# alexv879/ClusterMachineLearningForHospitalNetworks-Apache-Spark

Measured on AMD Instinct MI355X. Metric: KMeans fit samples/sec (whole node), 100M×256 k=256 at 1/2/4/8 MI355X, higher is better.
Workload: dtype bf16; 1 GPU; model=KMeans k=256, 100000000x256, global_batch=100000000, parallelism=dp1, k=256, rows=100000000, dim=256

## Files before the change

clustermachinelearningforhospitalnetworks_apache_spark_amd/_native/csrc/kmeans.hip:

```cpp
#include <algorithm>

#include "common.h"

namespace {

constexpr int kAccumThreads = 1024;
constexpr int kSegThreads = 256;

template <int DP>
struct AssignShape {
  static constexpr int NCH = DP / 8;
  static constexpr int KS = DP >= 32 ? DP / 32 : 1;
};
constexpr int kAssignThreads = 512;

template <bool HI>
__device__ __forceinline__ unsigned f8x2_to_bf16x2(unsigned w) {
  typedef float f2 __attribute__((ext_vector_type(2)));
  const f2 v = __builtin_amdgcn_cvt_pk_f32_fp8((int)w, HI);
  return (__float_as_uint(v.x) >> 16) | (__float_as_uint(v.y) & 0xffff0000u);
}

template <int DP, bool F8>
__device__ __forceinline__ void load_x16(const void* __restrict__ Xv, long long n, long long ldx, long long row0,
// ... 457 lines not shown
    msg[kd + c] = (double)tot[c];
    carry = base;
    if (c == k - 1) {
      seg[k] = (int)(base + tot[c]);
      double cs = 0.0;
      for (int i = 0; i < ncost; ++i) cs += cost_part[i];
      msg[kd + k] = cs;
    }
  }
  __syncthreads();
  for (int b0 = 0; b0 < nblk; b0 += blockDim.x) {
    const int b = b0 + tid;
    const long long v = b < nblk ? hist[(long long)b * kp + c] : 0;
    long long incl = v;
#pragma unroll
    for (int o = 1; o < 64; o <<= 1) {
      const long long y = __shfl_up(incl, o, 64);
      if (lane >= o) incl += y;
    }
    __syncthreads();
    if (lane == 63) ws[wave] = incl;
    __syncthreads();
    long long pre = carry;
    for (int w = 0; w < wave; ++w) pre += ws[w];
    if (b < nblk) off[(long long)c * nblk + b] = (int)(pre + incl - v);
    __syncthreads();
    if (tid == blockDim.x - 1) carry = pre + incl;
    __syncthreads();
  }
}

constexpr int kScatterThreads = 512;
constexpr int kScatterU = 4;
__global__ __launch_bounds__(kScatterThreads) void kmeans_scatter(const int* __restrict__ labels,
                                                                  const int* __restrict__ rank, long long n, int nblk,
                                                                  int nwaves, int tile_rows, int k,
                                                                  const int* __restrict__ off, int* __restrict__ perm,
                                                                  const int* __restrict__ gate, int want) {
  extern __shared__ int soff[];
  if (gate != nullptr && gate[0] != want) return;
  const int b = blockIdx.x;
  for (int c = threadIdx.x; c < k; c += blockDim.x) soff[c] = off[(long long)c * nblk + b];
  __syncthreads();
  const long long grp = (long long)nwaves * tile_rows;
  const long long stride = grp * nblk;
  const int per = (long long)blockDim.x >= grp ? (int)(blockDim.x / grp) : 1;
  const int ro = per > 1 ? (int)(threadIdx.x / grp) : 0;
  if (ro >= per) return;
  const long long o0 = per > 1 ? (long long)threadIdx.x - ro * grp : (long long)threadIdx.x;
  const long long ostep = per > 1 ? grp : (long long)blockDim.x;
  for (long long q0 = ro; (long long)b * grp + q0 * stride < n; q0 += (long long)per * kScatterU) {
    for (long long o = o0; o < grp; o += ostep) {
      int lab[kScatterU], rk[kScatterU];
      long long rows[kScatterU];
#pragma unroll
      for (int u = 0; u < kScatterU; ++u) {
        rows[u] = (long long)b * grp + (q0 + (long long)u * per) * stride + o;
        lab[u] = rows[u] < n ? labels[rows[u]] : -1;
        rk[u] = rows[u] < n ? rank[rows[u]] : 0;
      }
#pragma unroll
      for (int u = 0; u < kScatterU; ++u)
        if (lab[u] >= 0) {
          const long long pos = (long long)soff[lab[u]] + rk[u];
          if (pos < n) perm[pos] = (int)rows[u];
        }
    }
  }
}

template <int CPL> struct RawCols;
template <> struct RawCols<2> { using T = unsigned; };
template <> struct RawCols<4> { using T = uint2; };
template <> struct RawCols<8> { using T = uint4; };

template <int CPL>
__device__ __forceinline__ void add_raw(double (&acc)[CPL], const typename RawCols<CPL>::T& w) {
  const unsigned* ws = reinterpret_cast<const unsigned*>(&w);
#pragma unroll
  for (int q = 0; q < CPL / 2; ++q) {
    acc[2 * q] += (double)bf16_to_f32((u16)(ws[q] & 0xffffu));
    acc[2 * q + 1] += (double)bf16_to_f32((u16)(ws[q] >> 16));
  }
}

template <int CPL>
__device__ __forceinline__ void add_raw_q(double (&acc)[CPL], const typename RawCols<CPL>::T& w, double qs,
                                          float qsf) {
  const unsigned* ws = reinterpret_cast<const unsigned*>(&w);
  if (qsf != 0.f) {
#pragma unroll
    for (int q = 0; q < CPL / 2; ++q) {
      acc[2 * q] += (double)rintf(bf16_to_f32((u16)(ws[q] & 0xffffu)) * qsf);
      acc[2 * q + 1] += (double)rintf(bf16_to_f32((u16)(ws[q] >> 16)) * qsf);
    }
  } else {
#pragma unroll
    for (int q = 0; q < CPL / 2; ++q) {
      acc[2 * q] += rint((double)bf16_to_f32((u16)(ws[q] & 0xffffu)) * qs);
// ... 68 lines not shown
      s = fmaf(e0, e0, s);
      s = fmaf(e1, e1, s);
    }
  }
  return s;
}

__device__ __forceinline__ float wave_total_dpp(float v) {
  v += __int_as_float(__builtin_amdgcn_update_dpp(0, __float_as_int(v), 0xB1, 0xf, 0xf, false));
  v += __int_as_float(__builtin_amdgcn_update_dpp(0, __float_as_int(v), 0x4E, 0xf, 0xf, false));
  v += __int_as_float(__builtin_amdgcn_update_dpp(0, __float_as_int(v), 0x141, 0xf, 0xf, false));
  v += __int_as_float(__builtin_amdgcn_update_dpp(0, __float_as_int(v), 0x140, 0xf, 0xf, false));
  v += __int_as_float(__builtin_amdgcn_update_dpp(0, __float_as_int(v), 0x142, 0xa, 0xf, false));
  v += __int_as_float(__builtin_amdgcn_update_dpp(0, __float_as_int(v), 0x143, 0xc, 0xf, false));
  return __int_as_float(__builtin_amdgcn_readlane(__float_as_int(v), 63));
}

__device__ __forceinline__ float batch16_totals(const float (&s)[16]) {
  const int lane = threadIdx.x & 63;
  const bool h5 = lane & 32, h4 = lane & 16, h3 = lane & 8, h2 = lane & 4;
  float a[8], b[4], c[2];
#pragma unroll
  for (int i = 0; i < 8; ++i) a[i] = (h5 ? s[8 + i] : s[i]) + __shfl_xor(h5 ? s[i] : s[8 + i], 32, 64);
#pragma unroll
  for (int i = 0; i < 4; ++i) b[i] = (h4 ? a[4 + i] : a[i]) + __shfl_xor(h4 ? a[i] : a[4 + i], 16, 64);
#pragma unroll
  for (int i = 0; i < 2; ++i) c[i] = (h3 ? b[2 + i] : b[i]) + __shfl_xor(h3 ? b[i] : b[2 + i], 8, 64);
  float v = (h2 ? c[1] : c[0]) + __shfl_xor(h2 ? c[0] : c[1], 4, 64);
  v += __int_as_float(__builtin_amdgcn_update_dpp(0, __float_as_int(v), 0xB1, 0xf, 0xf, false));
  v += __int_as_float(__builtin_amdgcn_update_dpp(0, __float_as_int(v), 0x4E, 0xf, 0xf, false));
  return __shfl(v, 4 * (lane & 15), 64);
}

struct SegUB {
  const u16* cb;
  long long ldc;
  float* ub;
  double qs;
  const float* cu = nullptr;
};

__device__ __forceinline__ long long seg_chunk(long long filled, long long waves) {
  const long long c = (filled + waves - 1) / waves;
  return c > 128 ? c : 128;
}

template <int CPL, bool F8, bool UB = false, bool Q = false>
__global__ __launch_bounds__(kSegThreads, (CPL <= 4 ? 4 : 1)) void kmeans_segacc(const void* __restrict__ X, long long n, long long ldx,
                                                             int Dp, int D, const int* __restrict__ perm,
                                                             const int* __restrict__ seg, int k,
                                                             double* __restrict__ msg, double* __restrict__ slots,
                                                             int* __restrict__ slot_c, const int* __restrict__ gate,
                                                             int want, SegUB sub) {
  using raw_t = typename SegRaw<CPL, F8>::T;
  constexpr int U = 16;
  if (gate != nullptr && gate[0] != want) return;
  const unsigned char* xb = reinterpret_cast<const unsigned char*>(X);
  constexpr int ESZ = F8 ? 1 : 2;
  const int lane = threadIdx.x & 63;
  const long long wave = (long long)blockIdx.x * (kSegThreads / 64) + (threadIdx.x >> 6);
  n = n < (long long)seg[k] ? n : (long long)seg[k];
  const long long chunk = seg_chunk(n, (long long)gridDim.x * (kSegThreads / 64));
  const long long p0 = wave * chunk;
  if (p0 >= n) {
    if (lane == 0) {
      slot_c[2 * wave] = -1;
      slot_c[2 * wave + 1] = -1;
    }
    return;
  }
  double* slotA = slots + (2 * wave) * (long long)D;
  double* slotB = slotA + D;
  int nflush = 0;
  const long long p1 = p0 + chunk < n ? p0 + chunk : n;
  int lo = 0, hi = k;
  while (hi - lo > 1) {
    const int mid = (lo + hi) >> 1;
    if (seg[mid] <= p0) lo = mid; else hi = mid;
  }
  int c = lo;
  long long next = seg[c + 1];
  while (next <= p0) { ++c; next = seg[c + 1]; }
  const int col = CPL * lane;
  const bool active = col < Dp;
  double acc[CPL];
#pragma unroll
  for (int j = 0; j < CPL; ++j) acc[j] = 0.0;
  float cv[CPL];
  auto load_cv = [&](int cc) {
#pragma unroll
    for (int j = 0; j < CPL; ++j) cv[j] = active ? bf16_to_f32(sub.cb[(long long)cc * sub.ldc + col + j]) : 0.f;
  };
  if constexpr (UB) load_cv(c);
  const float qsf = grid_scale_f32(sub.qs);
  auto ub_of = [](float s) { return sqrtf(s * (1.0f + 1.0f / 8192.0f)) * (1.0f + 1e-6f); };
  auto ub_store = [&](float u, int cc) {
    if (sub.cu == nullptr) return u;
    const float cu = sub.cu[cc];
    return (u - cu) + 1e-6f * (u + cu);
  };
  int pr_next = (lane < U && p0 + lane < p1) ? perm[p0 + lane] : 0;
  for (long long p = p0; p < p1; p += U) {
    const int cnt = (int)(p1 - p < U ? p1 - p : U);
    const int pr = pr_next;
    pr_next = (lane < U && p + U + lane < p1) ? perm[p + U + lane] : 0;
    float mine = 0.f;
    raw_t w[U];
#pragma unroll
    for (int u = 0; u < U; ++u) {
      const long long row = __builtin_amdgcn_readlane(pr, u);
      if (u < cnt && active) {
        w[u] = *reinterpret_cast<const raw_t*>(xb + (row * ldx + col) * ESZ);
      } else {
        w[u] = raw_t{};
      }
    }
    const long long pe = p + cnt;
    if (next >= pe) {
      if constexpr (UB) {
        static_assert(U == 16, "batch16_totals");
        if constexpr (CPL <= 8) {
          float sq[U];
#pragma unroll
          for (int u = 0; u < U; ++u) sq[u] = sqdist_raw<CPL, F8>(w[u], cv);
          mine = batch16_totals(sq);
        } else {
#pragma unroll
          for (int u = 0; u < U; ++u) {
            const float t = wave_total_dpp(sqdist_raw<CPL, F8>(w[u], cv));
            mine = lane == u ? t : mine;
          }
        }
        if (lane < cnt) sub.ub[pr] = ub_store(ub_of(mine), c);
      }
      if constexpr (F8) {
        float part[CPL];
#pragma unroll
        for (int j = 0; j < CPL; ++j) part[j] = 0.f;
#pragma unroll
        for (int u = 0; u < U; ++u) add_raw8_f32<CPL>(part, w[u]);
#pragma unroll
        for (int j = 0; j < CPL; ++j) acc[j] += (double)part[j];
      } else {
#pragma unroll
        for (int u = 0; u < U; ++u) {
          if constexpr (Q) add_raw_q<CPL>(acc, w[u], sub.qs, qsf);
          else add_raw<CPL>(acc, w[u]);
        }
      }
    } else {
      int rc = c;
#pragma unroll 1
      for (int u = 0; u < cnt; ++u) {
        const long long pos = p + u;
        while (pos >= next) {
          double* dst = nflush == 0 ? slotA : msg + (long long)c * D;
          if (active) {
#pragma unroll
            for (int j = 0; j < CPL; ++j)
              if (col + j < D) dst[col + j] = acc[j];
          }
          if (nflush == 0 && lane == 0) slot_c[2 * wave] = c;
          ++nflush;
#pragma unroll
          for (int j = 0; j < CPL; ++j) acc[j] = 0.0;
          ++c;
          next = seg[c + 1];
          while (next <= pos && c < k - 1) { ++c; next = seg[c + 1]; }
          if constexpr (UB) load_cv(c);
        }
        const long long row = __builtin_amdgcn_readlane(pr, u);
        raw_t v = raw_t{};
        if (active) v = *reinterpret_cast<const raw_t*>(xb + (row * ldx + col) * ESZ);
        if constexpr (UB) {
          const float t = wave_total_dpp(sqdist_raw<CPL, F8>(v, cv));
          mine = lane == u ? t : mine;
          rc = lane == u ? c : rc;
        }
        if constexpr (F8) add_raw8<CPL>(acc, v);
        else if constexpr (Q) add_raw_q<CPL>(acc, v, sub.qs, qsf);
        else add_raw<CPL>(acc, v);
      }
      if constexpr (UB) {
        if (lane < cnt) sub.ub[pr] = ub_store(ub_of(mine), rc);
      }
    }
  }
  if (active) {
#pragma unroll
    for (int j = 0; j < CPL; ++j)
      if (col + j < D) slotB[col + j] = acc[j];
  }
  if (lane == 0) {
    if (nflush == 0) slot_c[2 * wave] = -1;
    slot_c[2 * wave + 1] = c;
  }
}

__device__ __forceinline__ float init_reach(float cost, float xn, float pn, float tau) {
  return 2.0f * sqrtf(fmaxf(cost, 0.f) + tau * (xn + pn)) * (1.0f + 2e-6f);
}

constexpr int kClsPer = 16;
constexpr int kClsRows = 256 * kClsPer;

__global__ __launch_bounds__(256) void init_classify_kernel(const float* __restrict__ cost,
                                                            const int* __restrict__ near, const float* __restrict__ xn,
                                                            const float* __restrict__ pn,
                                                            const float* __restrict__ tab_v, int m, float tau,
                                                            long long n, int lmax, int* __restrict__ list_a,
                                                            int* __restrict__ cnt_a, int* __restrict__ list_b,
                                                            int* __restrict__ cnt_b) {
  __shared__ int wa[4], wb[4], base[2];
  const int lane = threadIdx.x & 63, wv = threadIdx.x >> 6;
  for (long long c0 = (long long)blockIdx.x * kClsRows; c0 < n; c0 += (long long)gridDim.x * kClsRows) {
    unsigned cls = 0;
#pragma unroll
// ... 446 lines not shown
int launch_assign(const void* X, long long n, long long ldx, const u16* C, long long ldc, int kc, int kp,
                  int c_base, const float* cnorm, const float* xnorm, int* labels, float* best, int first, int last,
                  double* cost_part, int* hist, int* rank, DeltaOut dout, int grid, hipStream_t st) {
  const size_t lds = (size_t)assign_lds_bytes(kc, kp, DP);
  const void* fn = assign_kernel_ptr<DP, F8>();
  hipFuncSetAttribute(fn, hipFuncAttributeMaxDynamicSharedMemorySize, (int)lds);
  void* args[] = {(void*)&X, (void*)&n, (void*)&ldx, (void*)&C, (void*)&ldc, (void*)&kc, (void*)&kp,
                  (void*)&c_base, (void*)&cnorm, (void*)&xnorm, (void*)&labels, (void*)&best, (void*)&first,
                  (void*)&last, (void*)&cost_part, (void*)&hist, (void*)&rank, (void*)&dout};
  const hipError_t e = hipLaunchKernel(fn, dim3(grid), dim3(kAssignThreads), args, lds, st);
  if (e != hipSuccess) return (int)e;
  return cml_status();
}

long long priv_lds_bytes(int k, int dw, int rpw) {
  const long long NW = kAccumThreads / 64;
  return NW * rpw * k * dw * 4 + NW * rpw * k * 4;
}

template <int CPL, int RPW>
int launch_priv(const u16* X, long long n, long long ldx, const int* labels, int k, int dw, float* slab, int* cslab,
                int gx, int nsl, hipStream_t st) {
  const size_t lds = (size_t)priv_lds_bytes(k, dw, RPW);
  hipFuncSetAttribute((const void*)kmeans_accum_priv<CPL, RPW>, hipFuncAttributeMaxDynamicSharedMemorySize, (int)lds);
  hipLaunchKernelGGL((kmeans_accum_priv<CPL, RPW>), dim3(gx, nsl), dim3(kAccumThreads), lds, st, X, n, ldx, labels, k,
                     dw, slab, cslab);
  return cml_status();
}

int launch_segsum(const void* X, long long n, long long ldx, int Dp, int D, const int* perm, const int* seg, int k,
                  int cpl, int seg_grid, double* msg, double* slots, int* slot_c, int xfp8, const int* gate, int want,
                  hipStream_t st, SegUB sub = SegUB{nullptr, 0, nullptr, 0.0}, bool fixup = true) {
  const long long waves = (long long)seg_grid * (kSegThreads / 64);
#define CML_SEG_L(C, F, U, Q)                                                                                       \
  hipLaunchKernelGGL((kmeans_segacc<C, F, U, Q>), dim3(seg_grid), dim3(kSegThreads), 0, st, X, n, ldx, Dp, D, perm, \
                     seg, k, msg, slots, slot_c, gate, want, sub)
#define CML_SEG(C, F)                                                  \
  if (sub.ub != nullptr) {                                             \
    if (!F && sub.qs != 0.0) CML_SEG_L(C, F, true, !F);               \
    else CML_SEG_L(C, F, true, false);                                 \
  } else {                                                             \
    if (!F && sub.qs != 0.0) CML_SEG_L(C, F, false, !F);              \
    else CML_SEG_L(C, F, false, false);                                \
  }
  if (xfp8) {
    if (cpl == 4) CML_SEG(4, true)
    else if (cpl == 8) CML_SEG(8, true)
    else if (cpl == 16) CML_SEG(16, true)
    else return (int)hipErrorInvalidValue;
  } else if (cpl == 2) CML_SEG(2, false)
  else if (cpl == 4) CML_SEG(4, false)
  else if (cpl == 8) CML_SEG(8, false)
  else return (int)hipErrorInvalidValue;
#undef CML_SEG
#undef CML_SEG_L
  const int e = cml_status();
  if (e || !fixup) return e;
  hipLaunchKernelGGL(kmeans_seg_fixup, dim3(k), dim3(256), 0, st, seg, k, D, n, waves, slots, slot_c, msg, gate,
                     want);
  return cml_status();
}

}

CML_API long long cml_kmeans_assign_lds_bytes(int kc, int kp, int Dp) { return assign_lds_bytes(kc, kp, Dp); }
CML_API int cml_kmeans_assign_threads(int ) { return kAssignThreads; }
CML_API int cml_kmeans_assign_occupancy(int Dp, int kc, int kp, int xfp8) {
  if (xfp8) {
    switch (Dp) {
      case 64: return assign_occupancy<64, true>(kc, kp);
      case 128: return assign_occupancy<128, true>(kc, kp);
      case 256: return assign_occupancy<256, true>(kc, kp);
      case 512: return assign_occupancy<512, true>(kc, kp);
      default: return 0;
    }
  }
// ... 143 lines not shown
  CML_PRIV(2, 1); CML_PRIV(2, 2); CML_PRIV(2, 4); CML_PRIV(2, 8); CML_PRIV(2, 16);
  CML_PRIV(4, 1); CML_PRIV(4, 2); CML_PRIV(4, 4); CML_PRIV(4, 8); CML_PRIV(4, 16);
#undef CML_PRIV
  return (int)hipErrorInvalidValue;
}

CML_API int cml_kmeans_reduce(const float* slab, const int* cslab, const double* cost_part, int gx, int ncost, int k,
                              int D, int dsl, double* out, void* stream) {
  const long long total = (long long)k * D + k + 1;
  const int threads = 256;
  const long long blocks = (total + threads - 1) / threads;
  hipLaunchKernelGGL(kmeans_reduce_kernel, dim3((unsigned)blocks), dim3(threads), 0, (hipStream_t)stream, slab, cslab,
                     cost_part, gx, ncost, k, D, dsl, out);
  return cml_status();
}

static int sort_accum(const void* X, long long n, long long ldx, int Dp, int D, const int* labels, const int* rank,
                      const int* hist, int nblk, int round_rows, int k, int kp, const double* cost_part, int ncost,
                      int* off, int* seg, int* perm, int cpl, int seg_grid, double* msg, double* slots, int* slot_c,
                      int xfp8, const int* gate, void* stream, SegUB sub);
CML_API int cml_kmeans_sort_accum(const void* X, long long n, long long ldx, int Dp, int D, const int* labels,
                                  const int* rank, const int* hist, int nblk, int round_rows, int k, int kp,
                                  const double* cost_part, int ncost, int* off, int* seg, int* perm, int cpl,
                                  int seg_grid, double* msg, double* slots, int* slot_c, int xfp8, const int* gate,
                                  double qscale, void* stream) {
  return sort_accum(X, n, ldx, Dp, D, labels, rank, hist, nblk, round_rows, k, kp, cost_part, ncost, off, seg, perm,
                    cpl, seg_grid, msg, slots, slot_c, xfp8, gate, stream, SegUB{nullptr, 0, nullptr, qscale});
}
CML_API int cml_kmeans_sort_accum_ub(const void* X, long long n, long long ldx, int Dp, int D, const int* labels,
                                     const int* rank, const int* hist, int nblk, int round_rows, int k, int kp,
                                     const double* cost_part, int ncost, int* off, int* seg, int* perm, int cpl,
                                     int seg_grid, double* msg, double* slots, int* slot_c, int xfp8, const int* gate,
                                     const void* cb, long long ldc, float* ub, double qscale, const float* cu,
                                     void* stream) {
  if (cb == nullptr || ub == nullptr || ldc < Dp) return (int)hipErrorInvalidValue;
  return sort_accum(X, n, ldx, Dp, D, labels, rank, hist, nblk, round_rows, k, kp, cost_part, ncost, off, seg, perm,
                    cpl, seg_grid, msg, slots, slot_c, xfp8, gate, stream, SegUB{(const u16*)cb, ldc, ub, qscale, cu});
}
static int sort_accum(const void* X, long long n, long long ldx, int Dp, int D, const int* labels, const int* rank,
                      const int* hist, int nblk, int round_rows, int k, int kp, const double* cost_part, int ncost,
                      int* off, int* seg, int* perm, int cpl, int seg_grid, double* msg, double* slots, int* slot_c,
                      int xfp8, const int* gate, void* stream, SegUB sub) {
  hipStream_t st = (hipStream_t)stream;
  long long* tot = reinterpret_cast<long long*>(seg + k + 1 + ((k + 1) & 1));
  const int want = 1;
  if (gate == nullptr) {
    hipMemsetAsync(msg, 0, sizeof(double) * (size_t)k * D, st);
  } else {
    hipLaunchKernelGGL(zero_f64_gated, dim3(256), dim3(256), 0, st, msg, (long long)k * D, gate, want);
  }
  hipLaunchKernelGGL(kmeans_seg_totals, dim3(k), dim3(256), 0, st, hist, nblk, kp, tot, gate, want);
  hipLaunchKernelGGL(kmeans_seg_offsets, dim3(k), dim3(256), 0, st, hist, nblk, k, kp, tot, cost_part, ncost, D, off,
                     seg, msg, gate, want);
  int e = cml_status();
  if (e) return e;
  if (n == 0) return 0;
  hipLaunchKernelGGL(kmeans_scatter, dim3(nblk), dim3(kScatterThreads), sizeof(int) * (size_t)k, st,
                     labels, rank, n,
                     nblk, 1, round_rows, k, off, perm, gate, want);
  e = cml_status();
  if (e) return e;
  return launch_segsum(X, n, ldx, Dp, D, perm, seg, k, cpl, seg_grid, msg, slots, slot_c, xfp8, gate, want, st, sub);
}

CML_API int cml_kmeans_sort_perm(long long n, const int* labels, const int* rank, const int* hist, int nblk,
                                 int round_rows, int k, int kp, const double* cost_part, int ncost, int* off, int* seg,
                                 int* perm, double* tail, void* stream) {
  if (k <= 0 || nblk <= 0 || n < 0 || tail == nullptr) return (int)hipErrorInvalidValue;
  hipStream_t st = (hipStream_t)stream;
  long long* tot = reinterpret_cast<long long*>(seg + k + 1 + ((k + 1) & 1));
  hipLaunchKernelGGL(kmeans_seg_totals, dim3(k), dim3(256), 0, st, hist, nblk, kp, tot, (const int*)nullptr, 1);
  hipLaunchKernelGGL(kmeans_seg_offsets, dim3(k), dim3(256), 0, st, hist, nblk, k, kp, tot, cost_part,
                     cost_part != nullptr ? ncost : 0, 0, off, seg, tail, (const int*)nullptr, 1);
  int e = cml_status();
  if (e || n == 0) return e;
  hipLaunchKernelGGL(kmeans_scatter, dim3(nblk), dim3(kScatterThreads), sizeof(int) * (size_t)k, st, labels, rank, n,
                     nblk, 1, round_rows, k, off, perm, (const int*)nullptr, 1);
  return cml_status();
}

CML_API int cml_kmeans_delta_gate(const int* chg_wg_count, int nblk, int cap, int* chg_overflow, int* force, int* mode,
                                  int k, int* dh, void* stream) {
  hipLaunchKernelGGL(kmeans_delta_gate, dim3(1), dim3(256), 0, (hipStream_t)stream, chg_wg_count, nblk, cap,
                     chg_overflow, force, mode, k, dh);
  return cml_status();
}

CML_API int cml_kmeans_delta_accum(const void* X, long long ldx, int Dp, int D, const int* labels, const int* chg_rows,
                                   const int* chg_old, const int* chg_wg_count, int nblk, int pcap, int cap,
                                   const int* mode, int k, int* dh, int* dseg,
                                   int* cursor, int* dperm, int cpl, int seg_grid, double* dsum, double* slots,
                                   int* slot_c, double* acc, const double* cost_part, int ncost, double* msg, int xfp8,
                                   double qscale, void* stream) {
  hipStream_t st = (hipStream_t)stream;
  const size_t lh = sizeof(int) * 2 * (size_t)k;
  hipLaunchKernelGGL(kmeans_delta_hist, dim3(nblk), dim3(kDeltaThreads), lh, st, chg_rows, chg_old, labels,
                     chg_wg_count, pcap, mode, k, dh, dsum, 2LL * k * D, cursor);
  hipLaunchKernelGGL(kmeans_delta_scatter, dim3(nblk), dim3(kDeltaThreads), lh + sizeof(int) * (2 * (size_t)k + 1), st,
                     chg_rows, chg_old, labels, chg_wg_count, pcap, mode, k, cursor, dperm, dh, dseg);
  int e = cml_status();
  if (e) return e;
  if (cap > 0) {
    e = launch_segsum(X, 2LL * cap, ldx, Dp, D, dperm, dseg, 2 * k, cpl, seg_grid, dsum, slots, slot_c, xfp8, mode, 0,
                      st, SegUB{nullptr, 0, nullptr, qscale}, false);
    if (e) return e;
  }
  const long long total = (long long)k * D + k + 1;
  const long long waves = (long long)seg_grid * (kSegThreads / 64);
  hipLaunchKernelGGL(kmeans_delta_apply, dim3((unsigned)((total + 255) / 256)), dim3(256), 0, st, acc, dsum, dseg,
                     mode, k, D, cost_part, ncost, msg, cap > 0 ? slots : nullptr, slot_c, 2LL * cap, waves);
// ... 61 lines not shown
```

clustermachinelearningforhospitalnetworks_apache_spark_amd/models/kmeans.py:

```python
from __future__ import annotations

import math
import os
import types
from typing import List, Optional

import numpy as np
import torch

from .. import _native
from ..ops import kmeans_ops as K
from ..ops.group_ops import group_reduce
from ..parallel.comm import Communicator, local_comm
from ..utils import rng
from ..utils.device import padded_dim, round_up
from ..utils.fault import maybe_fail
from ..utils.trace import trace


def padded_dim_fp8(d: int) -> int:
    return max(256, 1 << max(0, (d - 1).bit_length()))


def to_device_matrix(x: torch.Tensor, d: Optional[int] = None) -> torch.Tensor:
# ... 1006 lines not shown
        if self._conv_lim is not None:
            K.converge_latch(self.shift2, k, self._conv_lim, st.flags)

    def _seed_from_init(self, sd) -> None:
        st, n, k, d = self._pst, self.n, self.k, self.d
        if n == 0:
            return
        U = sd.uniq.to(device=self.device, dtype=torch.float64)
        a, d1, d2, pn32 = K.seed_table(U, self.cb, k)
        qmap = sd.inverse.reshape(-1).to(torch.int32).contiguous()
        if st.cum is not None:
            st.cum.zero_()
        K.seed_bounds(sd.nearest[:n], sd.costs[:n], self.xnorm[:n], qmap, a, d1, d2, pn32, 2.0 * self._tau, n,
                      self.labels[:n], st.ub[:n], st.lb[:n])

    def _step_seeded(self) -> None:
        st, dl = self._pst, self.delta
        n, k, d, ap = self.n, self.k, self.d, self.aplan
        x, lab, msg = self.x, self.labels, self.msgs[0]
        if n:
            K.prune_bounds(lab, st.ub, st.lb, st.drift, st.dmax, st.thr, st.c2, k, st.cand, st.count,
                           xn=self.xnorm, cand_lab=st.cand_lab, cand_xn=st.cand_xn, zero_count=True, cum=st.cum)
            K.prune_gate(st.count, st.cap_m, st.flags, st.pmode)
            K.assign_rr_ext(1, x, n, self.dp, self.cb, self.cnorm, ap, self.xnorm, lab, self.cost_part, st.ub, st.lb,
                            st.mc, st.tau, hist=self.hist, rank=self.rank, delta=dl, gate=st.pmode, want=1,
                            cum=st.cum)
            K.assign_rr_ext(2, x, st.cap_m, self.dp, self.cb, self.cnorm, ap, st.cand_xn, lab, None, st.ub, st.lb,
                            st.mc, st.tau, delta=dl, idx=st.cand, n_dev=st.count, lab_in=st.cand_lab, gate=st.pmode,
                            want=0, cum=st.cum)
            K.label_hist(lab, n, ap, self.hist, self.rank, gate=st.pmode, want=0)
        self.cost_part.zero_()
        dl.invalidate()
        dl.gate(0)
        K.accumulate_sort(x, n, self.dp, d, lab, self.rank, self.hist, ap, k, self.cost_part, self.off, self.seg,
                          self.perm, self.cplan, dl.acc[0], self.slots, gate=dl.mode[0],
                          ub_centres=self.cb, ub=st.ub, qscale=self._qscale, cum=st.cum)
        dl.accumulate(x, self.dp, lab, 0, self.cost_part, ap.grid, msg, qscale=self._qscale)
        self.comm.allreduce_async(msg).wait()
        self._pdev_post()

    def _norms64(self) -> torch.Tensor:
        self._ensure_norms()
        if self._xnorm64 is None:
            self._xnorm64 = torch.empty(max(self.n, 1), dtype=torch.float64, device=self.device)
            if self.n:
                tmp = torch.empty(self.n, dtype=torch.float32, device=self.device)
                for _, r0, r1, xc in self._x_chunks(whole=True):
                    K.row_pass(xc, r1 - r0, self.dp, tmp[r0:r1], xn64=self._xnorm64[r0:r1])
        return self._xnorm64

    def _device_cost(self) -> torch.Tensor:
        k, d, n = self.k, self.d, self.n
        cb = self._pst.cb_cost if self._pdev else self._cb_cost
        if k <= 4096:
            bound = self._xmax_dev()
            limbs = torch.zeros(2 * k, dtype=torch.int64, device=self.device)
            if n:
                lab = self.labels[:n]
                lab = lab if lab.dtype == torch.int32 and lab.is_contiguous() else lab.to(torch.int32).contiguous()
                K.fixsum(self._norms64()[:n], n, bound, 1.0, lab=lab, k=k, limbs=limbs)
            self.comm.allreduce_(limbs)
            q = K.fixsum_finalize(limbs, k, bound, 1.0)
        else:
            if n:
                q = group_reduce(self.labels[:n], self._norms64()[:n], k, "sum",
                                 ids_in_range=True).to(torch.float64).contiguous()
            else:
                q = torch.zeros(k, dtype=torch.float64, device=self.device)
            self.comm.allreduce_(q)
# ... 829 lines not shown
```

clustermachinelearningforhospitalnetworks_apache_spark_amd/ops/kmeans_ops.py:

```python
from __future__ import annotations

import ctypes
import os
import threading

from dataclasses import dataclass

import torch

from .. import _native
from .._native import c_dbl, c_int, c_ll, c_vp
from ..utils.device import LDS_BUDGET, num_cus, round_up

_native.register_kernel_sigs({
    "cml_kmeans_assign_lds_bytes": (c_ll, [c_int, c_int, c_int]),
    "cml_kmeans_assign_threads": (c_int, [c_int]),
    "cml_kmeans_set_assign_variant": (c_int, [c_int]),
    "cml_kmeans_assign_occupancy": (c_int, [c_int, c_int, c_int, c_int]),
    "cml_kmeans_seg_threads": (c_int, []),
    "cml_kmeans_seg_ints": (c_ll, [c_int]),
    "cml_kmeans_assign_bf16": (c_int, [c_vp, c_ll, c_ll, c_int, c_vp, c_ll, c_int, c_int, c_int, c_vp, c_vp, c_vp,
                                       c_vp, c_int, c_int, c_vp, c_vp, c_vp, c_int, c_int, c_vp, c_vp, c_vp, c_vp,
                                       c_int, c_int, c_vp]),
    "cml_kmeans_assign_rr_plan": (c_int, [c_int, c_int, c_int, c_int, c_vp]),
    "cml_kmeans_set_rr_default": (c_int, [c_int]),
    "cml_kmeans_set_rr_debug": (c_int, [c_int]),
    "cml_kmeans_set_rr_m32": (c_int, [c_int]),
    "cml_kmeans_set_fp8_mx": (c_int, [c_int]),
    "cml_kmeans_assign_tile_rows": (c_int, [c_int]),
    "cml_row_sqnorm_bf16": (c_int, [c_vp, c_ll, c_ll, c_int, c_vp, c_vp]),
    "cml_row_sqnorm_fp8": (c_int, [c_vp, c_ll, c_ll, c_int, c_vp, c_vp]),
    "cml_kmeans_priv_lds_bytes": (c_ll, [c_int, c_int, c_int]),
    "cml_kmeans_accum_priv": (c_int, [c_vp, c_ll, c_ll, c_vp, c_int, c_int, c_int, c_int, c_vp, c_vp, c_int, c_int,
                                      c_vp]),
    "cml_kmeans_reduce": (c_int, [c_vp, c_vp, c_vp, c_int, c_int, c_int, c_int, c_int, c_vp, c_vp]),
    "cml_kmeans_sort_accum": (c_int, [c_vp, c_ll, c_ll, c_int, c_int, c_vp, c_vp, c_vp, c_int, c_int, c_int, c_int,
                                      c_vp, c_int, c_vp, c_vp, c_vp, c_int, c_int, c_vp, c_vp, c_vp, c_int, c_vp,
                                      ctypes.c_double, c_vp]),
    "cml_kmeans_sort_accum_ub": (c_int, [c_vp, c_ll, c_ll, c_int, c_int, c_vp, c_vp, c_vp, c_int, c_int, c_int,
                                         c_int, c_vp, c_int, c_vp, c_vp, c_vp, c_int, c_int, c_vp, c_vp, c_vp, c_int,
                                         c_vp, c_vp, c_ll, c_vp, ctypes.c_double, c_vp, c_vp]),
    "cml_kmeans_delta_gate": (c_int, [c_vp, c_int, c_int, c_vp, c_vp, c_vp, c_int, c_vp, c_vp]),
    "cml_kmeans_delta_accum": (c_int, [c_vp, c_ll, c_int, c_int, c_vp, c_vp, c_vp, c_vp, c_int, c_int, c_int, c_vp,
                                       c_int, c_vp, c_vp, c_vp, c_vp, c_int, c_int, c_vp, c_vp, c_vp, c_vp, c_vp,
                                       c_int, c_vp, c_int, ctypes.c_double, c_vp]),
    "cml_kmeans_seg_slot_doubles": (c_ll, [c_int, c_int]),
    "cml_kmeans_seg_slot_ints": (c_ll, [c_int]),
    "cml_kmeans_update": (c_int, [c_vp, c_int, c_ll, c_int, c_int, c_vp, c_vp, c_ll, c_int, c_int, c_vp, c_vp,
                                  ctypes.c_double, c_vp]),
    "cml_kmeans_prune_lower": (c_int, [c_vp, c_int, c_vp, c_vp, ctypes.c_float, ctypes.c_float, c_ll, c_vp, c_vp]),
    "cml_kmeans_prune_bounds": (c_int, [c_vp, c_vp, c_vp, c_vp, c_vp, c_vp, c_vp, c_int, c_ll, c_vp,
                                        c_vp, c_vp, c_vp, c_vp, c_vp, c_ll, c_vp, c_vp]),
    "cml_kmeans_prune_gate": (c_int, [c_vp, c_ll, c_vp, c_vp, c_vp, c_int, c_vp]),
    "cml_kmeans_converge_latch": (c_int, [c_vp, c_int, ctypes.c_double, c_vp, c_vp]),
    "cml_kmeans_cond_copy": (c_int, [c_vp, c_vp, c_ll, c_vp, c_vp, c_vp]),
    "cml_kmeans_seed_bounds": (c_int, [c_vp, c_vp, c_vp, c_vp, c_vp, c_vp, c_vp, c_vp, ctypes.c_float, c_ll,
                                       c_vp, c_vp, c_vp, c_vp]),
    "cml_kmeans_label_hist": (c_int, [c_vp, c_ll, c_int, c_int, c_int, c_vp, c_vp, c_vp, c_int, c_vp]),
    "cml_kmeans_centre_stats": (c_int, [c_vp, c_vp, c_ll, c_int, c_int, c_vp, ctypes.c_float, c_vp, c_vp, c_vp,
                                        c_vp, c_vp, c_vp, c_vp, c_vp, c_vp, c_vp, c_vp, c_vp]),
    "cml_kmeans_assign_rr_ext": (c_int, [c_int, c_vp, c_ll, c_ll, c_int, c_vp, c_ll, c_int, c_int, c_vp, c_vp,
                                         c_vp, c_vp, c_vp, c_vp, c_int, c_int, c_vp, c_vp, c_vp, c_vp, c_int,
                                         c_int, c_vp, c_vp, c_vp, c_vp, c_vp, c_vp, ctypes.c_float, c_vp, c_int,
                                         c_vp, c_vp, c_int, c_vp, c_vp, c_int, c_vp]),
    "cml_kmeans_init_classify": (c_int, [c_vp, c_vp, c_vp, c_vp, c_vp, c_int, ctypes.c_float, c_ll, c_int, c_vp,
                                         c_vp, c_vp, c_vp, c_vp]),
    "cml_kmeans_init_near_list": (c_int, [c_vp, c_ll, c_int, c_int, c_vp, c_vp, c_vp, c_vp, c_vp, c_vp, c_int, c_vp,
                                          c_int, ctypes.c_float, c_vp, c_vp, c_ll, c_vp]),
    "cml_kmeans_init_merge_list": (c_int, [c_vp, c_vp, c_vp, c_vp, c_int, c_vp, c_vp, c_ll, c_vp]),
})


_native.register_kernel_sigs({
    "cml_kmeans_row_pass": (c_int, [c_vp, c_ll, c_ll, c_int, c_int, c_vp, c_vp, ctypes.c_float, c_vp, c_vp, c_vp,
# ... 433 lines not shown
    return out


def accumulate_priv(x: torch.Tensor, n: int, labels: torch.Tensor, k: int, plan: AccumPlan,
                    slab: torch.Tensor, cslab: torch.Tensor, stream=None) -> None:
    lib = _native.kernels()
    status = lib.cml_kmeans_accum_priv(x.data_ptr(), n, x.stride(0), labels.data_ptr(), k, plan.dw, plan.cpl,
                                       plan.rpw, slab.data_ptr(), cslab.data_ptr(), plan.gx, plan.nsl,
                                       _native.stream_ptr(stream))
    _native.check(status, "kmeans_accum_priv")


def reduce_slabs(slab, cslab, cost_part, ncost: int, k: int, d: int, plan: AccumPlan, out: torch.Tensor,
                 stream=None) -> None:
    lib = _native.kernels()
    status = lib.cml_kmeans_reduce(slab.data_ptr(), cslab.data_ptr(), cost_part.data_ptr(), plan.gx, ncost, k,
                                   d, plan.dsl, out.data_ptr(), _native.stream_ptr(stream))
    _native.check(status, "kmeans_reduce")


def seg_slots(plan: AccumPlan, d: int, device) -> tuple:
    lib = _native.kernels()
    sl = torch.empty(max(int(lib.cml_kmeans_seg_slot_doubles(plan.seg_grid, d)), 1), dtype=torch.float64,
                     device=device)
    sc = torch.empty(max(int(lib.cml_kmeans_seg_slot_ints(plan.seg_grid)), 1), dtype=torch.int32, device=device)
    return sl, sc


def accumulate_sort(x: torch.Tensor, n: int, dp: int, d: int, labels: torch.Tensor, rank: torch.Tensor,
                    hist: torch.Tensor, aplan: AssignPlan, k: int, cost_part: torch.Tensor, off: torch.Tensor,
                    seg: torch.Tensor, perm: torch.Tensor, plan: AccumPlan, msg: torch.Tensor,
                    slots: tuple, stream=None, gate: torch.Tensor | None = None,
                    ub_centres: torch.Tensor | None = None, ub: torch.Tensor | None = None,
                    qscale: float = 0.0, cum: torch.Tensor | None = None) -> None:
    lib = _native.kernels()
    args = (x.data_ptr(), n, x.stride(0), dp, d, labels.data_ptr(), rank.data_ptr(), hist.data_ptr(), aplan.grid,
            aplan.round_rows, k, aplan.kp, cost_part.data_ptr(), aplan.grid, off.data_ptr(), seg.data_ptr(),
            perm.data_ptr(), plan.cpl, plan.seg_grid, msg.data_ptr(), slots[0].data_ptr(), slots[1].data_ptr(),
            int(is_fp8(x)), gate.data_ptr() if gate is not None else 0)
    if ub is not None:
        if ub_centres is None or ub_centres.dtype != torch.bfloat16 or ub.dtype != torch.float32 or ub.numel() < n:
            raise ValueError("accumulate_sort: ub needs bf16 centres and an f32 [n] output")
        status = lib.cml_kmeans_sort_accum_ub(*args, ub_centres.data_ptr(), ub_centres.stride(0), ub.data_ptr(),
                                              float(qscale), _ptr(cum), _native.stream_ptr(stream))
    else:
        status = lib.cml_kmeans_sort_accum(*args, float(qscale), _native.stream_ptr(stream))
    _native.check(status, "kmeans_sort_accum")


def sort_perm(labels: torch.Tensor, rank: torch.Tensor, hist: torch.Tensor, aplan: AssignPlan, n: int, k: int,
              off: torch.Tensor, seg: torch.Tensor, perm: torch.Tensor, tail: torch.Tensor | None = None,
              cost_part: torch.Tensor | None = None, stream=None) -> torch.Tensor:
    i32 = torch.int32
    if any(t.dtype != i32 or not t.is_contiguous() for t in (labels, rank, hist, off, seg, perm)):
        raise ValueError("sort_perm: contiguous int32 labels, rank, hist, off, seg and perm")
    if (labels.numel() < n or rank.numel() < n or perm.numel() < n or hist.numel() < aplan.grid * aplan.kp
            or off.numel() < k * aplan.grid or seg.numel() < seg_buffer_ints(k) or k > aplan.kp):
        raise ValueError("sort_perm: buffer lengths do not match n, k and the assign plan")
    if tail is None:
        tail = torch.empty(k + 1, dtype=torch.float64, device=labels.device)
    elif tail.dtype != torch.float64 or tail.numel() < k + 1 or not tail.is_contiguous():
        raise ValueError("sort_perm: tail is a contiguous f64 [k + 1] tensor")
    if cost_part is not None and (cost_part.dtype != torch.float64 or cost_part.numel() < aplan.grid):
        raise ValueError("sort_perm: cost_part is the assign's f64 [grid] tensor")
    _native.check(_native.kernels().cml_kmeans_sort_perm(
        int(n), labels.data_ptr(), rank.data_ptr(), hist.data_ptr(), aplan.grid, aplan.round_rows, int(k), aplan.kp,
        _ptr(cost_part), aplan.grid, off.data_ptr(), seg.data_ptr(), perm.data_ptr(), tail.data_ptr(),
        _native.stream_ptr(stream)), "kmeans_sort_perm")
    return tail


def wseg_slots(plan: AccumPlan, d: int, device) -> tuple:
    lib = _native.kernels()
    sl = torch.empty(max(int(lib.cml_kmeans_wseg_slot_doubles(plan.seg_grid, d)), 1), dtype=torch.float64,
                     device=device)
    sc = torch.empty(max(int(lib.cml_kmeans_wseg_slot_ints(plan.seg_grid)), 1), dtype=torch.int32, device=device)
    return sl, sc


def _weighted_columns(x: torch.Tensor, n: int, d: int, w: torch.Tensor, xn64: torch.Tensor) -> torch.Tensor:
    xs = x[:n, :d]
    x64 = (xs.to(torch.float32) if is_fp8(xs) else xs).to(torch.float64)
    w = w[:n].to(torch.float64)
    return torch.cat([x64 * w[:, None], w[:, None], (w * xn64[:n].to(torch.float64))[:, None]], 1)


def weighted_sums(x: torch.Tensor, n: int, dp: int, d: int, w: torch.Tensor, xn64: torch.Tensor, k: int,
                  perm: torch.Tensor, seg: torch.Tensor, plan: AccumPlan | None = None,
                  out: tuple | None = None, slots: tuple | None = None, stream=None) -> tuple:
    if w.dtype != torch.float64 or xn64.dtype != torch.float64 or not w.is_contiguous() or not xn64.is_contiguous():
        raise ValueError("weighted_sums: w and xn64 are contiguous f64 vectors")
    if w.numel() < n or xn64.numel() < n or x.shape[0] < n:
        raise ValueError("weighted_sums: w, xn64 and x need n rows")
    if perm.dtype != torch.int32 or seg.dtype != torch.int32 or not perm.is_contiguous() or not seg.is_contiguous():
        raise ValueError("weighted_sums: perm and seg are contiguous int32 tensors")
    if perm.numel() < n or seg.numel() < k + 1:
        raise ValueError("weighted_sums: perm [n] and seg [k + 1]")
    if not x.is_cuda:
        lab = torch.empty(n, dtype=torch.int64)
        sizes = (seg[1:k + 1] - seg[:k]).long()
        lab[perm[:n].long()] = torch.repeat_interleave(torch.arange(k), sizes)
        S, _, S_lo = sums_reference(_weighted_columns(x, n, d, w, xn64), lab, k, with_lo=True)
# ... 690 lines not shown
```

Baseline: 115.2 billion samples/s.

## Write segment upper bounds in sorted order and unsort with a gather pass

The segmented accumulate kernel now writes per-row upper bounds contiguously into a sorted-order scratch buffer instead of scattering them to random row indices. A second pass of the scatter kernel, templated for unsorting, gathers them back into row order with coalesced writes. The wave reduction for the squared distance also switches to a cheaper shuffle-tree variant for small column counts. This trades random scattered stores for an extra pass and a scratch buffer, which is enabled by default through an environment variable.

```diff
diff --git a/clustermachinelearningforhospitalnetworks_apache_spark_amd/_native/csrc/kmeans.hip b/clustermachinelearningforhospitalnetworks_apache_spark_amd/_native/csrc/kmeans.hip
--- a/clustermachinelearningforhospitalnetworks_apache_spark_amd/_native/csrc/kmeans.hip
+++ b/clustermachinelearningforhospitalnetworks_apache_spark_amd/_native/csrc/kmeans.hip
@@ -513,10 +513,13 @@
 
 constexpr int kScatterThreads = 512;
 constexpr int kScatterU = 4;
+template <bool UNSORT>
 __global__ __launch_bounds__(kScatterThreads) void kmeans_scatter(const int* __restrict__ labels,
                                                                   const int* __restrict__ rank, long long n, int nblk,
                                                                   int nwaves, int tile_rows, int k,
                                                                   const int* __restrict__ off, int* __restrict__ perm,
+                                                                  const float* __restrict__ src,
+                                                                  float* __restrict__ dst,
                                                                   const int* __restrict__ gate, int want) {
   extern __shared__ int soff[];
   if (gate != nullptr && gate[0] != want) return;
@@ -540,12 +543,26 @@
         lab[u] = rows[u] < n ? labels[rows[u]] : -1;
         rk[u] = rows[u] < n ? rank[rows[u]] : 0;
       }
-#pragma unroll
-      for (int u = 0; u < kScatterU; ++u)
-        if (lab[u] >= 0) {
-          const long long pos = (long long)soff[lab[u]] + rk[u];
-          if (pos < n) perm[pos] = (int)rows[u];
+      if constexpr (UNSORT) {
+        float v[kScatterU];
+        bool ok[kScatterU];
+#pragma unroll
+        for (int u = 0; u < kScatterU; ++u) {
+          const long long pos = lab[u] >= 0 ? (long long)soff[lab[u]] + rk[u] : n;
+          ok[u] = pos < n;
+          v[u] = ok[u] ? src[pos] : 0.f;
         }
+#pragma unroll
+        for (int u = 0; u < kScatterU; ++u)
+          if (ok[u]) dst[rows[u]] = v[u];
+      } else {
+#pragma unroll
+        for (int u = 0; u < kScatterU; ++u)
+          if (lab[u] >= 0) {
+            const long long pos = (long long)soff[lab[u]] + rk[u];
+            if (pos < n) perm[pos] = (int)rows[u];
+          }
+      }
     }
   }
 }
@@ -680,12 +697,23 @@
   return __shfl(v, 4 * (lane & 15), 64);
 }
 
+__device__ __forceinline__ float wave_total_b16(float v) {
+  v += __shfl_xor(v, 32, 64);
+  v += __shfl_xor(v, 16, 64);
+  v += __shfl_xor(v, 8, 64);
+  v += __shfl_xor(v, 4, 64);
+  v += __int_as_float(__builtin_amdgcn_update_dpp(0, __float_as_int(v), 0xB1, 0xf, 0xf, false));
+  v += __int_as_float(__builtin_amdgcn_update_dpp(0, __float_as_int(v), 0x4E, 0xf, 0xf, false));
+  return v;
+}
+
 struct SegUB {
   const u16* cb;
   long long ldc;
   float* ub;
   double qs;
   const float* cu = nullptr;
+  float* ub_sorted = nullptr;
 };
 
 __device__ __forceinline__ long long seg_chunk(long long filled, long long waves) {
@@ -693,7 +721,7 @@
   return c > 128 ? c : 128;
 }
 
-template <int CPL, bool F8, bool UB = false, bool Q = false>
+template <int CPL, bool F8, bool UB = false, bool Q = false, bool UBS = false>
 __global__ __launch_bounds__(kSegThreads, (CPL <= 4 ? 4 : 1)) void kmeans_segacc(const void* __restrict__ X, long long n, long long ldx,
                                                              int Dp, int D, const int* __restrict__ perm,
                                                              const int* __restrict__ seg, int k,
@@ -747,6 +775,10 @@
     const float cu = sub.cu[cc];
     return (u - cu) + 1e-6f * (u + cu);
   };
+  auto ub_put = [&](long long p, int row, float v) {
+    if constexpr (UBS) (sub.ub_sorted + p)[(unsigned)lane] = v;
+    else sub.ub[row] = v;
+  };
   int pr_next = (lane < U && p0 + lane < p1) ? perm[p0 + lane] : 0;
   for (long long p = p0; p < p1; p += U) {
     const int cnt = (int)(p1 - p < U ? p1 - p : U);
@@ -779,7 +811,7 @@
             mine = lane == u ? t : mine;
           }
         }
-        if (lane < cnt) sub.ub[pr] = ub_store(ub_of(mine), c);
+        if (lane < cnt) ub_put(p, pr, ub_store(ub_of(mine), c));
       }
       if constexpr (F8) {
         float part[CPL];
@@ -821,7 +853,8 @@
         raw_t v = raw_t{};
         if (active) v = *reinterpret_cast<const raw_t*>(xb + (row * ldx + col) * ESZ);
         if constexpr (UB) {
-          const float t = wave_total_dpp(sqdist_raw<CPL, F8>(v, cv));
+          const float sq = sqdist_raw<CPL, F8>(v, cv);
+          const float t = CPL <= 8 ? wave_total_b16(sq) : wave_total_dpp(sq);
           mine = lane == u ? t : mine;
           rc = lane == u ? c : rc;
         }
@@ -830,7 +863,7 @@
         else add_raw<CPL>(acc, v);
       }
       if constexpr (UB) {
-        if (lane < cnt) sub.ub[pr] = ub_store(ub_of(mine), rc);
+        if (lane < cnt) ub_put(p, pr, ub_store(ub_of(mine), rc));
       }
     }
   }
@@ -1343,16 +1376,19 @@
                   int cpl, int seg_grid, double* msg, double* slots, int* slot_c, int xfp8, const int* gate, int want,
                   hipStream_t st, SegUB sub = SegUB{nullptr, 0, nullptr, 0.0}, bool fixup = true) {
   const long long waves = (long long)seg_grid * (kSegThreads / 64);
-#define CML_SEG_L(C, F, U, Q)                                                                                       \
-  hipLaunchKernelGGL((kmeans_segacc<C, F, U, Q>), dim3(seg_grid), dim3(kSegThreads), 0, st, X, n, ldx, Dp, D, perm, \
-                     seg, k, msg, slots, slot_c, gate, want, sub)
+#define CML_SEG_L(C, F, U, Q, S)                                                                                  \
+  hipLaunchKernelGGL((kmeans_segacc<C, F, U, Q, S>), dim3(seg_grid), dim3(kSegThreads), 0, st, X, n, ldx, Dp, D,  \
+                     perm, seg, k, msg, slots, slot_c, gate, want, sub)
 #define CML_SEG(C, F)                                                  \
-  if (sub.ub != nullptr) {                                             \
-    if (!F && sub.qs != 0.0) CML_SEG_L(C, F, true, !F);               \
-    else CML_SEG_L(C, F, true, false);                                 \
+  if (sub.ub != nullptr && sub.ub_sorted != nullptr) {                 \
+    if (!F && sub.qs != 0.0) CML_SEG_L(C, F, true, !F, true);         \
+    else CML_SEG_L(C, F, true, false, true);                           \
+  } else if (sub.ub != nullptr) {                                      \
+    if (!F && sub.qs != 0.0) CML_SEG_L(C, F, true, !F, false);        \
+    else CML_SEG_L(C, F, true, false, false);                          \
   } else {                                                             \
-    if (!F && sub.qs != 0.0) CML_SEG_L(C, F, false, !F);              \
-    else CML_SEG_L(C, F, false, false);                                \
+    if (!F && sub.qs != 0.0) CML_SEG_L(C, F, false, !F, false);       \
+    else CML_SEG_L(C, F, false, false, false);                         \
   }
   if (xfp8) {
     if (cpl == 4) CML_SEG(4, true)
@@ -1562,10 +1598,11 @@
                                      const double* cost_part, int ncost, int* off, int* seg, int* perm, int cpl,
                                      int seg_grid, double* msg, double* slots, int* slot_c, int xfp8, const int* gate,
                                      const void* cb, long long ldc, float* ub, double qscale, const float* cu,
-                                     void* stream) {
-  if (cb == nullptr || ub == nullptr || ldc < Dp) return (int)hipErrorInvalidValue;
+                                     float* ub_sorted, void* stream) {
+  if (cb == nullptr || ub == nullptr || ldc < Dp || ub_sorted == ub) return (int)hipErrorInvalidValue;
   return sort_accum(X, n, ldx, Dp, D, labels, rank, hist, nblk, round_rows, k, kp, cost_part, ncost, off, seg, perm,
-                    cpl, seg_grid, msg, slots, slot_c, xfp8, gate, stream, SegUB{(const u16*)cb, ldc, ub, qscale, cu});
+                    cpl, seg_grid, msg, slots, slot_c, xfp8, gate, stream,
+                    SegUB{(const u16*)cb, ldc, ub, qscale, cu, ub_sorted});
 }
 static int sort_accum(const void* X, long long n, long long ldx, int Dp, int D, const int* labels, const int* rank,
                       const int* hist, int nblk, int round_rows, int k, int kp, const double* cost_part, int ncost,
@@ -1585,12 +1622,29 @@
   int e = cml_status();
   if (e) return e;
   if (n == 0) return 0;
-  hipLaunchKernelGGL(kmeans_scatter, dim3(nblk), dim3(kScatterThreads), sizeof(int) * (size_t)k, st,
+  hipLaunchKernelGGL(kmeans_scatter<false>, dim3(nblk), dim3(kScatterThreads), sizeof(int) * (size_t)k, st,
                      labels, rank, n,
-                     nblk, 1, round_rows, k, off, perm, gate, want);
+                     nblk, 1, round_rows, k, off, perm, (const float*)nullptr, (float*)nullptr, gate, want);
   e = cml_status();
   if (e) return e;
-  return launch_segsum(X, n, ldx, Dp, D, perm, seg, k, cpl, seg_grid, msg, slots, slot_c, xfp8, gate, want, st, sub);
+  e = launch_segsum(X, n, ldx, Dp, D, perm, seg, k, cpl, seg_grid, msg, slots, slot_c, xfp8, gate, want, st, sub);
+  if (e || sub.ub_sorted == nullptr) return e;
+  hipLaunchKernelGGL(kmeans_scatter<true>, dim3(nblk), dim3(kScatterThreads), sizeof(int) * (size_t)k, st, labels,
+                     rank, n, nblk, 1, round_rows, k, off, (int*)nullptr, (const float*)sub.ub_sorted, sub.ub, gate,
+                     want);
+  return cml_status();
+}
+
+CML_API int cml_kmeans_unsort_f32(long long n, const int* labels, const int* rank, int nblk, int round_rows, int k,
+                                  const int* off, const float* src, float* dst, const int* gate, int want,
+                                  void* stream) {
+  if (k <= 0 || nblk <= 0 || round_rows <= 0 || n < 0 || src == nullptr || dst == nullptr)
+    return (int)hipErrorInvalidValue;
+  if (n == 0) return 0;
+  hipLaunchKernelGGL(kmeans_scatter<true>, dim3(nblk), dim3(kScatterThreads), sizeof(int) * (size_t)k,
+                     (hipStream_t)stream, labels, rank, n, nblk, 1, round_rows, k, off, (int*)nullptr, src, dst, gate,
+                     want);
+  return cml_status();
 }
 
 CML_API int cml_kmeans_sort_perm(long long n, const int* labels, const int* rank, const int* hist, int nblk,
@@ -1604,8 +1658,9 @@
                      cost_part != nullptr ? ncost : 0, 0, off, seg, tail, (const int*)nullptr, 1);
   int e = cml_status();
   if (e || n == 0) return e;
-  hipLaunchKernelGGL(kmeans_scatter, dim3(nblk), dim3(kScatterThreads), sizeof(int) * (size_t)k, st, labels, rank, n,
-                     nblk, 1, round_rows, k, off, perm, (const int*)nullptr, 1);
+  hipLaunchKernelGGL(kmeans_scatter<false>, dim3(nblk), dim3(kScatterThreads), sizeof(int) * (size_t)k, st, labels,
+                     rank, n, nblk, 1, round_rows, k, off, perm, (const float*)nullptr, (float*)nullptr,
+                     (const int*)nullptr, 1);
   return cml_status();
 }
 
diff --git a/clustermachinelearningforhospitalnetworks_apache_spark_amd/models/kmeans.py b/clustermachinelearningforhospitalnetworks_apache_spark_amd/models/kmeans.py
--- a/clustermachinelearningforhospitalnetworks_apache_spark_amd/models/kmeans.py
+++ b/clustermachinelearningforhospitalnetworks_apache_spark_amd/models/kmeans.py
@@ -1062,9 +1062,14 @@
         self.cost_part.zero_()
         dl.invalidate()
         dl.gate(0)
+        ub_sorted = None
+        if n and os.environ.get("CML_KMEANS_SEG_UB", "sorted") != "scatter":
+            sc = self._iscr
+            ub_sorted = sc.best if sc is not None and sc.best.numel() >= n else torch.empty(
+                n, dtype=torch.float32, device=self.device)
         K.accumulate_sort(x, n, self.dp, d, lab, self.rank, self.hist, ap, k, self.cost_part, self.off, self.seg,
                           self.perm, self.cplan, dl.acc[0], self.slots, gate=dl.mode[0],
-                          ub_centres=self.cb, ub=st.ub, qscale=self._qscale, cum=st.cum)
+                          ub_centres=self.cb, ub=st.ub, qscale=self._qscale, cum=st.cum, ub_sorted=ub_sorted)
         dl.accumulate(x, self.dp, lab, 0, self.cost_part, ap.grid, msg, qscale=self._qscale)
         self.comm.allreduce_async(msg).wait()
         self._pdev_post()
diff --git a/clustermachinelearningforhospitalnetworks_apache_spark_amd/ops/kmeans_ops.py b/clustermachinelearningforhospitalnetworks_apache_spark_amd/ops/kmeans_ops.py
--- a/clustermachinelearningforhospitalnetworks_apache_spark_amd/ops/kmeans_ops.py
+++ b/clustermachinelearningforhospitalnetworks_apache_spark_amd/ops/kmeans_ops.py
@@ -39,7 +39,8 @@
                                       ctypes.c_double, c_vp]),
     "cml_kmeans_sort_accum_ub": (c_int, [c_vp, c_ll, c_ll, c_int, c_int, c_vp, c_vp, c_vp, c_int, c_int, c_int,
                                          c_int, c_vp, c_int, c_vp, c_vp, c_vp, c_int, c_int, c_vp, c_vp, c_vp, c_int,
-                                         c_vp, c_vp, c_ll, c_vp, ctypes.c_double, c_vp, c_vp]),
+                                         c_vp, c_vp, c_ll, c_vp, ctypes.c_double, c_vp, c_vp, c_vp]),
+    "cml_kmeans_unsort_f32": (c_int, [c_ll, c_vp, c_vp, c_int, c_int, c_int, c_vp, c_vp, c_vp, c_vp, c_int, c_vp]),
     "cml_kmeans_delta_gate": (c_int, [c_vp, c_int, c_int, c_vp, c_vp, c_vp, c_int, c_vp, c_vp]),
     "cml_kmeans_delta_accum": (c_int, [c_vp, c_ll, c_int, c_int, c_vp, c_vp, c_vp, c_vp, c_int, c_int, c_int, c_vp,
                                        c_int, c_vp, c_vp, c_vp, c_vp, c_int, c_int, c_vp, c_vp, c_vp, c_vp, c_vp,
@@ -539,7 +540,8 @@
                     seg: torch.Tensor, perm: torch.Tensor, plan: AccumPlan, msg: torch.Tensor,
                     slots: tuple, stream=None, gate: torch.Tensor | None = None,
                     ub_centres: torch.Tensor | None = None, ub: torch.Tensor | None = None,
-                    qscale: float = 0.0, cum: torch.Tensor | None = None) -> None:
+                    qscale: float = 0.0, cum: torch.Tensor | None = None,
+                    ub_sorted: torch.Tensor | None = None) -> None:
     lib = _native.kernels()
     args = (x.data_ptr(), n, x.stride(0), dp, d, labels.data_ptr(), rank.data_ptr(), hist.data_ptr(), aplan.grid,
             aplan.round_rows, k, aplan.kp, cost_part.data_ptr(), aplan.grid, off.data_ptr(), seg.data_ptr(),
@@ -548,9 +550,14 @@
     if ub is not None:
         if ub_centres is None or ub_centres.dtype != torch.bfloat16 or ub.dtype != torch.float32 or ub.numel() < n:
             raise ValueError("accumulate_sort: ub needs bf16 centres and an f32 [n] output")
+        if ub_sorted is not None and (ub_sorted.dtype != torch.float32 or ub_sorted.numel() < n
+                                      or not ub_sorted.is_contiguous() or ub_sorted.data_ptr() == ub.data_ptr()):
+            raise ValueError("accumulate_sort: ub_sorted is a contiguous f32 [n] scratch other than ub")
         status = lib.cml_kmeans_sort_accum_ub(*args, ub_centres.data_ptr(), ub_centres.stride(0), ub.data_ptr(),
-                                              float(qscale), _ptr(cum), _native.stream_ptr(stream))
+                                              float(qscale), _ptr(cum), _ptr(ub_sorted), _native.stream_ptr(stream))
     else:
+        if ub_sorted is not None:
+            raise ValueError("accumulate_sort: ub_sorted without ub")
         status = lib.cml_kmeans_sort_accum(*args, float(qscale), _native.stream_ptr(stream))
     _native.check(status, "kmeans_sort_accum")
 
@@ -575,6 +582,21 @@
         _ptr(cost_part), aplan.grid, off.data_ptr(), seg.data_ptr(), perm.data_ptr(), tail.data_ptr(),
         _native.stream_ptr(stream)), "kmeans_sort_perm")
     return tail
+
+
+def unsort_f32(src: torch.Tensor, dst: torch.Tensor, labels: torch.Tensor, rank: torch.Tensor, aplan: AssignPlan,
+               n: int, k: int, off: torch.Tensor, stream=None, gate: torch.Tensor | None = None,
+               want: int = 1) -> None:
+    if (src.dtype != torch.float32 or dst.dtype != torch.float32 or not src.is_contiguous()
+            or not dst.is_contiguous() or src.numel() < n or dst.numel() < n or src.data_ptr() == dst.data_ptr()):
+        raise ValueError("unsort_f32: src and dst are distinct contiguous f32 [n] tensors")
+    if any(t.dtype != torch.int32 or not t.is_contiguous() for t in (labels, rank, off)):
+        raise ValueError("unsort_f32: contiguous int32 labels, rank and off")
+    if labels.numel() < n or rank.numel() < n or off.numel() < k * aplan.grid:
+        raise ValueError("unsort_f32: buffer lengths do not match n, k and the assign plan")
+    _native.check(_native.kernels().cml_kmeans_unsort_f32(
+        int(n), labels.data_ptr(), rank.data_ptr(), aplan.grid, aplan.round_rows, int(k), off.data_ptr(),
+        src.data_ptr(), dst.data_ptr(), _ptr(gate), int(want), _native.stream_ptr(stream)), "kmeans_unsort_f32")
 
 
 def wseg_slots(plan: AccumPlan, d: int, device) -> tuple:
```

Result: slower. 113.0 billion samples/s (-1.9%).
